# kaushik87599/Melo-GAN

Measured on AMD Instinct MI355X. Metric: piano-roll samples/sec (G+D step), batch=64 128x256 roll, higher is better.
Workload: dtype f32; 1 GPU; cfg2: 128x256 piano-roll, batch=64 per GPU, full G+D+emotion-D step (1 critic update incl. gradient penalty + 1 generator update); global_batch=64, T=256, C=128, parallelism=dp1, graph=True

## Files before the change

### melo-gan_amd/csrc/small_kernels.hip

```cpp
#include "common.h"

namespace {

constexpr int RED_SPLITS = 256;

__device__ __forceinline__ float wave_sum(float v) {
#pragma unroll
    for (int o = 32; o > 0; o >>= 1) v += __shfl_xor(v, o, 64);
    return v;
}

__device__ __forceinline__ float block_sum(float v, float* sh) {
    v = wave_sum(v);
    const int w = threadIdx.x >> 6;
    __syncthreads();
    if ((threadIdx.x & 63) == 0) sh[w] = v;
    __syncthreads();
    float t = 0.f;
    for (int i = 0; i < (int)(blockDim.x >> 6); ++i) t += sh[i];
    return t;
}

template <int MODE>
__global__ __launch_bounds__(256) void colsum_partial_kernel(const float* __restrict__ x, const float* __restrict__ a,
// ... 97 lines not shown
    __shared__ double sh[2][16][FIN_CH];
    const int cx = threadIdx.x & (FIN_CH - 1), g = threadIdx.x / FIN_CH;
    const int c = blockIdx.x * FIN_CH + cx;
    double a = 0.0, b = 0.0;
    if (c < C)
        for (int k = g; k < nsplit; k += 16) {
            a += part[((long)k * 2) * C + c];
            if (want2) b += part[((long)k * 2 + 1) * C + c];
        }
    sh[0][g][cx] = a;
    sh[1][g][cx] = b;
    __syncthreads();
    c_out = c;
    if (g != 0 || c >= C) return false;
    s1 = 0.0;
    s2 = 0.0;
#pragma unroll
    for (int y = 0; y < 16; ++y) {
        s1 += sh[0][y][cx];
        s2 += sh[1][y][cx];
    }
    return true;
}

__global__ __launch_bounds__(256) void colsum_final_kernel(const double* __restrict__ part, int nsplit, int C,
                                                           float* sum, float* sumsq) {
    double s1, s2;
    int c;
    if (!reduce_partials(part, nsplit, C, sumsq != nullptr, s1, s2, c)) return;
    sum[c] = (float)s1;
    if (sumsq) sumsq[c] = (float)s2;
}

__global__ void bn_eval_kernel(const float* __restrict__ z, float* __restrict__ a, long n, int C,
                               const float* __restrict__ gamma, const float* __restrict__ beta,
                               const float* __restrict__ rm, const float* __restrict__ rv, float eps, int act) {
    const long i = (long)blockIdx.x * blockDim.x + threadIdx.x;
    if (i >= n) return;
    const int c = (int)(i % C);
    const float v = (z[i] - rm[c]) / sqrtf(rv[c] + eps) * gamma[c] + beta[c];
    a[i] = mg_act(act, v);
}

__global__ void bn_fold_kernel(const float* gamma, const float* beta, const float* rm, const float* rv,
                               const float* cb, float eps, float* scale, float* shift, int C) {
    const int c = blockIdx.x * blockDim.x + threadIdx.x;
    if (c >= C) return;
    const float s = gamma[c] / sqrtf(rv[c] + eps);
    scale[c] = s;
    shift[c] = beta[c] + ((cb ? cb[c] : 0.f) - rm[c]) * s;
}

constexpr int BNA_THREADS = 1024, BNA_PL = BNA_THREADS / 64;
__device__ __forceinline__ void combine_parts64(const float* __restrict__ part, int np, int C, int c0, double (*sh)[64],
                                                double& mean, double& var) {
    const int cx = threadIdx.x & 63, pl = threadIdx.x >> 6;
    double A = 0.0, Q = 0.0, Bt = 0.0, n = 0.0;
    if (c0 + cx < C) {
        for (int q0 = pl; q0 < np; q0 += 8 * BNA_PL) {
            float va[8], vq[8], vn[8];
#pragma unroll
            for (int j = 0; j < 8; ++j) {
                const int q = q0 + BNA_PL * j;
                const long o = ((long)(q < np ? q : np - 1) * 3) * C + c0 + cx;
                va[j] = part[o];
                vq[j] = part[o + C];
                vn[j] = part[o + 2 * (long)C];
            }
#pragma unroll
            for (int j = 0; j < 8; ++j)
                if (q0 + BNA_PL * j < np && vn[j] > 0.f) {
                    const double a = (double)va[j], c = (double)vn[j];
                    A += a; Q += (double)vq[j]; Bt += a * a / c; n += c;
                }
        }
    }
    __syncthreads();
    sh[pl][cx] = A; sh[BNA_PL + pl][cx] = Q; sh[2 * BNA_PL + pl][cx] = Bt; sh[3 * BNA_PL + pl][cx] = n;
    __syncthreads();
    A = Q = Bt = n = 0.0;
#pragma unroll
    for (int l = 0; l < BNA_PL; ++l) {
        A += sh[l][cx]; Q += sh[BNA_PL + l][cx]; Bt += sh[2 * BNA_PL + l][cx]; n += sh[3 * BNA_PL + l][cx];
    }
    mean = n > 0.0 ? A / n : 0.0;
    double m2 = Q + (Bt - A * mean);
    if (m2 < 0.0) m2 = 0.0;
    var = n > 0.0 ? m2 / n : 0.0;
}

__device__ __forceinline__ void combine_colsum64(const double* __restrict__ part, int np, int C, int c0, long R, double (*sh)[64],
                                                 double& mean, double& var) {
    const int cx = threadIdx.x & 63, pl = threadIdx.x >> 6;
    double A = 0.0, Q = 0.0;
    if (c0 + cx < C)
        for (int q0 = pl; q0 < np; q0 += 8 * BNA_PL) {
            double va[8], vq[8];
#pragma unroll
            for (int j = 0; j < 8; ++j) {
                const int q = q0 + BNA_PL * j;
                const long o = ((long)(q < np ? q : np - 1) * 2) * C + c0 + cx;
                va[j] = part[o];
                vq[j] = part[o + C];
            }
#pragma unroll
            for (int j = 0; j < 8; ++j)
                if (q0 + BNA_PL * j < np) { A += va[j]; Q += vq[j]; }
        }
    __syncthreads();
    sh[pl][cx] = A; sh[BNA_PL + pl][cx] = Q;
    __syncthreads();
    A = Q = 0.0;
#pragma unroll
    for (int l = 0; l < BNA_PL; ++l) { A += sh[l][cx]; Q += sh[BNA_PL + l][cx]; }
    mean = A / (double)R;
    var = Q / (double)R - mean * mean;
    if (var < 0.0) var = 0.0;
}

template <typename PT>
__global__ __launch_bounds__(BNA_THREADS) void bn_parts_apply_kernel(const PT* __restrict__ part, int np, int groups, long R, int C,
                                                             float momentum, float eps, float* running_mean, float* running_var,
                                                             float* save_mean, float* save_invstd, const float* __restrict__ z,
                                                             float* __restrict__ a, const float* __restrict__ gamma,
                                                             const float* __restrict__ beta, int act, long rows_per, int al16) {
    __shared__ double sh[4 * BNA_PL][64];
    __shared__ float s_mean[64], s_istd[64];
    const int c0 = blockIdx.x * 64, cx = threadIdx.x & 63;
    const int g = blockIdx.z;
    if (blockIdx.y == 0 && g == 0) {
        for (int gg = 0; gg < groups; ++gg) {
            double mean, var;
            if constexpr (sizeof(PT) == 4) combine_parts64(part + (long)gg * np * 3 * C, np, C, c0, sh, mean, var);
            else combine_colsum64(part + (long)gg * (RED_SPLITS + 1) * 2 * C, np, C, c0, R, sh, mean, var);
            if (threadIdx.x < 64 && c0 + cx < C) {
                const float mf = (float)mean, isf = (float)(1.0 / sqrt(var + (double)eps));
                save_mean[(long)gg * C + c0 + cx] = mf;
                save_invstd[(long)gg * C + c0 + cx] = isf;
                if (gg == 0) { s_mean[cx] = mf; s_istd[cx] = isf; }
                if (running_mean) {
                    const double unb = R > 1 ? var * (double)R / (double)(R - 1) : var;
                    running_mean[c0 + cx] = (float)((1.0 - momentum) * running_mean[c0 + cx] + momentum * mean);
                    running_var[c0 + cx] = (float)((1.0 - momentum) * running_var[c0 + cx] + momentum * unb);
                }
            }
        }
    } else {
        double mean, var;
        if constexpr (sizeof(PT) == 4) combine_parts64(part + (long)g * np * 3 * C, np, C, c0, sh, mean, var);
        else combine_colsum64(part + (long)g * (RED_SPLITS + 1) * 2 * C, np, C, c0, R, sh, mean, var);
        if (threadIdx.x < 64 && c0 + cx < C) {
            s_mean[cx] = (float)mean;
            s_istd[cx] = (float)(1.0 / sqrt(var + (double)eps));
        }
    }
    __syncthreads();
    const int cq = threadIdx.x & 15, ry = threadIdx.x >> 4;
    constexpr int RYN = BNA_THREADS / 16;
    const int c = c0 + 4 * cq;
    if (c >= C) return;
    const long r0 = (long)blockIdx.y * rows_per;
    long r1 = r0 + rows_per;
    if (r1 > R) r1 = R;
    const bool vec = al16 && (c + 3 < C);
    double mu[4], is[4], ga[4], be[4];
#pragma unroll
    for (int e = 0; e < 4; ++e) {
        const bool in = c + e < C;
        mu[e] = (double)s_mean[4 * cq + e];
        is[e] = (double)s_istd[4 * cq + e];
        ga[e] = in ? (double)gamma[c + e] : 0.0;
        be[e] = in ? (double)beta[c + e] : 0.0;
    }
    const float* zg = z + (long)g * R * C;
    float* ag = a + (long)g * R * C;
    for (long r = r0 + ry; r < r1; r += RYN) {
        const long i = r * C + c;
        if (vec) {
            const float4 t = *reinterpret_cast<const float4*>(zg + i);
            const float zv[4] = {t.x, t.y, t.z, t.w};
            float o[4];
#pragma unroll
            for (int e = 0; e < 4; ++e) o[e] = (float)(((double)zv[e] - mu[e]) * is[e] * ga[e] + be[e]);
            if (act == MG_ACT_RELU) {
#pragma unroll
                for (int e = 0; e < 4; ++e) o[e] = mg_act(MG_ACT_RELU, o[e]);
            } else if (act != MG_ACT_NONE) {
#pragma unroll
                for (int e = 0; e < 4; ++e) o[e] = mg_act(act, o[e]);
            }
            *reinterpret_cast<float4*>(ag + i) = make_float4(o[0], o[1], o[2], o[3]);
        } else {
            for (int e = 0; e < 4; ++e)
                if (c + e < C) ag[i + e] = mg_act(act, (float)(((double)zg[i + e] - mu[e]) * is[e] * ga[e] + be[e]));
        }
    }
}

template <typename PT>
__global__ __launch_bounds__(BNA_THREADS) void bn_bwd_parts_apply_kernel(const PT* __restrict__ part, int nsplit, int C, long R,
                                                                 const float* __restrict__ da, const float* __restrict__ a,
                                                                 const float* __restrict__ z, float* __restrict__ dz,
                                                                 const float* __restrict__ gamma, const float* __restrict__ beta,
                                                                 const float* __restrict__ mean, const float* __restrict__ invstd,
                                                                 float* dgamma, float* dbeta, int act, long rows_per, int al16) {
    __shared__ double sh[2 * BNA_PL][64];
    __shared__ double s1[64], s2[64];
    const int c0 = blockIdx.x * 64, cx = threadIdx.x & 63, pl = threadIdx.x >> 6;
    {
        double t1 = 0.0, t2 = 0.0;
        if (c0 + cx < C)
            for (int q0 = pl; q0 < nsplit; q0 += 8 * BNA_PL) {
                PT va[8], vb[8];
#pragma unroll
                for (int j = 0; j < 8; ++j) {
                    const int q = q0 + BNA_PL * j;
                    const long o = ((long)(q < nsplit ? q : nsplit - 1) * 2) * C + c0 + cx;
                    va[j] = part[o];
                    vb[j] = part[o + C];
                }
#pragma unroll
                for (int j = 0; j < 8; ++j)
                    if (q0 + BNA_PL * j < nsplit) { t1 += (double)va[j]; t2 += (double)vb[j]; }
            }
        sh[pl][cx] = t1;
        sh[BNA_PL + pl][cx] = t2;
        __syncthreads();
        if (threadIdx.x < 64) {
            double u1 = 0.0, u2 = 0.0;
#pragma unroll
            for (int l = 0; l < BNA_PL; ++l) { u1 += sh[l][cx]; u2 += sh[BNA_PL + l][cx]; }
            s1[cx] = u1;
            s2[cx] = u2;
            if (blockIdx.y == 0 && c0 + cx < C) {
                dbeta[c0 + cx] = (float)u1;
                dgamma[c0 + cx] = (float)u2;
            }
        }
        __syncthreads();
    }
    const int cq = threadIdx.x & 15, ry = threadIdx.x >> 4;
    constexpr int RYN = BNA_THREADS / 16;
    const int c = c0 + 4 * cq;
    if (c >= C) return;
    const long r0 = (long)blockIdx.y * rows_per;
    long r1 = r0 + rows_per;
    if (r1 > R) r1 = R;
    const bool vec = al16 && (c + 3 < C);
    const bool pre = act == MG_ACT_GELU;
    const double invR = 1.0 / (double)R;
    double mu[4], is[4], ga[4], be[4], k1[4], k2[4];
#pragma unroll
    for (int e = 0; e < 4; ++e) {
        const bool in = c + e < C;
        mu[e] = in ? (double)mean[c + e] : 0.0;
        is[e] = in ? (double)invstd[c + e] : 0.0;
        ga[e] = in ? (double)gamma[c + e] : 0.0;
        be[e] = (in && pre) ? (double)beta[c + e] : 0.0;
        k1[e] = s1[4 * cq + e];
        k2[e] = s2[4 * cq + e];
    }
    for (long r = r0 + ry; r < r1; r += RYN) {
        const long i = r * C + c;
        float dv[4] = {0, 0, 0, 0}, av[4] = {0, 0, 0, 0}, zv[4] = {0, 0, 0, 0};
        if (vec) {
            const float4 t = *reinterpret_cast<const float4*>(da + i);
            const float4 ta = *reinterpret_cast<const float4*>(a + i);
            const float4 tz = *reinterpret_cast<const float4*>(z + i);
            dv[0] = t.x; dv[1] = t.y; dv[2] = t.z; dv[3] = t.w;
            av[0] = ta.x; av[1] = ta.y; av[2] = ta.z; av[3] = ta.w;
            zv[0] = tz.x; zv[1] = tz.y; zv[2] = tz.z; zv[3] = tz.w;
        } else {
            for (int e = 0; e < 4; ++e)
                if (c + e < C) { dv[e] = da[i + e]; av[e] = a[i + e]; zv[e] = z[i + e]; }
        }
        float o[4];
#pragma unroll
        for (int e = 0; e < 4; ++e) {
            const double xh = ((double)zv[e] - mu[e]) * is[e];
            const float ref = pre ? (float)(xh * ga[e] + be[e]) : av[e];
            const double dy = (double)(dv[e] * mg_act_grad(act, ref));
            o[e] = (float)(ga[e] * is[e] * (dy - k1[e] * invR - xh * k2[e] * invR));
        }
        if (vec) *reinterpret_cast<float4*>(dz + i) = make_float4(o[0], o[1], o[2], o[3]);
        else
            for (int e = 0; e < 4; ++e)
                if (c + e < C) dz[i + e] = o[e];
    }
}

__global__ __launch_bounds__(256) void meanT_fwd_kernel(const float* __restrict__ a, float* __restrict__ h, int T, int C) {
    const int b = blockIdx.y;
    const int cq = threadIdx.x & 15, ry = threadIdx.x >> 4;
    const int c0 = blockIdx.x * 64 + 4 * cq;
    __shared__ float sh[16][65];
    float s[4] = {0.f, 0.f, 0.f, 0.f};
    const bool vec = ((C & 3) == 0) && ((((uintptr_t)a) & 15) == 0);
    if (c0 < C) {
        for (int t = ry; t < T; t += 16) {
            const float* row = a + ((long)b * T + t) * C + c0;
            if (vec) {
                const float4 v = *reinterpret_cast<const float4*>(row);
                s[0] += v.x; s[1] += v.y; s[2] += v.z; s[3] += v.w;
            } else {
                for (int e = 0; e < 4; ++e)
                    if (c0 + e < C) s[e] += row[e];
            }
        }
    }
#pragma unroll
    for (int e = 0; e < 4; ++e) sh[ry][4 * cq + e] = s[e];
    __syncthreads();
    if (threadIdx.x < 64) {
        const int c = blockIdx.x * 64 + threadIdx.x;
        if (c < C) {
            float t = 0.f;
#pragma unroll
            for (int y = 0; y < 16; ++y) t += sh[y][threadIdx.x];
            h[(long)b * C + c] = t / (float)T;
        }
    }
}

template <bool VEC>
__global__ void meanT_bwd_kernel(const float* __restrict__ dh, float* __restrict__ dz, long n, int T, int C,
                                 const float* __restrict__ gref, int gact, const float* __restrict__ gscale,
                                 const float* __restrict__ mean_src, float* mean_out, int mean_n, float mean_scale) {
    constexpr int NV = VEC ? 4 : 1;
    if (mean_out && blockIdx.x == gridDim.x - 1) {
        __shared__ float sh[16];
        float r = 0.f;
        for (int b = threadIdx.x; b < mean_n; b += blockDim.x) r += mean_src[b];
        r = block_sum(r, sh);
        if (threadIdx.x == 0) mean_out[0] = mean_scale * r / (float)mean_n;
        return;
    }
    const long i = ((long)blockIdx.x * blockDim.x + threadIdx.x) * NV;
    if (i >= n) return;
    const int c = (int)(i % C);
    const long b = i / ((long)T * C);
// ... 703 lines not shown
#pragma unroll
    for (int u = 0; u < AUG_UNROLL; ++u) {
        const int e = e0 + u * AUG_THREADS;
        if (e < n) d[e] = v[u];
    }
}

__global__ __launch_bounds__(256) void weighted_order_kernel(const double* __restrict__ cdf, long n, int64_t* __restrict__ order,
                                                             long m, unsigned long long seed, unsigned long long epoch) {
    const long i = (long)blockIdx.x * blockDim.x + threadIdx.x;
    if (i >= m) return;
    unsigned c[4];
    aug_draw(c, (unsigned)i, AUG_ORDER, epoch, seed);
    const unsigned long long bits = ((unsigned long long)(c[0] >> 5) << 26) | (unsigned long long)(c[1] >> 6);
    const double x = (double)bits * (1.0 / 9007199254740992.0) * cdf[n - 1];
    long lo = 0, hi = n - 1;
    while (lo < hi) {
        const long mid = (lo + hi) >> 1;
        if (cdf[mid] > x) hi = mid;
        else lo = mid + 1;
    }
    order[i] = lo < n - 1 ? lo : n - 1;
}

__global__ __launch_bounds__(64) void ed_metrics_acc_kernel(const float* __restrict__ logits, const int64_t* __restrict__ labels,
                                                            const float* __restrict__ loss, int rows, int C,
                                                            float* __restrict__ acc) {
    float hits = 0.f;
    for (int r = threadIdx.x; r < rows; r += 64) {
        const float* z = logits + (long)r * C;
        float mx = z[0];
        int am = 0;
        for (int j = 1; j < C; ++j) {
            const float v = z[j];
            if (v > mx || (isnan(v) && !isnan(mx))) { mx = v; am = j; }
        }
        hits += (long)am == labels[r] ? 1.f : 0.f;
    }
    hits = wave_sum(hits);
    if (threadIdx.x == 0) {
        acc[0] = __fadd_rn(acc[0], __fmul_rn(loss[0], (float)rows));
        acc[1] = __fadd_rn(acc[1], hits);
    }
}

__global__ void adam_advance_kernel(double* state, double beta1, double beta2) {
    if (threadIdx.x == 0 && blockIdx.x == 0) {
        if (state[0] == 0.0) { state[1] = 1.0; state[2] = 1.0; }
        state[0] += 1.0;
        state[1] *= beta1;
        state[2] *= beta2;
    }
}
struct WqTable { mg_wq_entry e[MG_MAX_WQ_ENTRIES]; int n; long lo, hi; };

__global__ void adam_apply_kernel(float* __restrict__ p, const float* __restrict__ g, float* __restrict__ m,
                                  float* __restrict__ v, long n, float lr, float beta1, float beta2, float eps,
                                  float wd, const double* __restrict__ state, float grad_scale,
                                  const float* __restrict__ gs_dev, unsigned long long* bump, const WqTable wq) {
    const long i = (long)blockIdx.x * blockDim.x + threadIdx.x;
    if (bump && i == 0) bump[0] += 1;
    if (i >= n) return;
    const double bc1 = 1.0 - state[1];
    const double bc2 = 1.0 - state[2];
    const float step_size = (float)((double)lr / bc1);
    const float bc2_sqrt = (float)sqrt(bc2);
    float gs = grad_scale;
    if (gs_dev) gs *= gs_dev[0];
    const float gi = g[i] * gs;
    float pi = p[i];
    if (wd != 0.f) pi *= (1.f - lr * wd);
    const float mi = m[i] + (gi - m[i]) * (1.f - beta1);
    const float vi = v[i] * beta2 + (1.f - beta2) * gi * gi;
    m[i] = mi;
    v[i] = vi;
    const float denom = sqrtf(vi) / bc2_sqrt + eps;
    pi = pi - step_size * (mi / denom);
    p[i] = pi;
    if (i >= wq.lo && i < wq.hi) {
        for (int t = 0; t < wq.n; ++t) {
            const mg_wq_entry& e = wq.e[t];
            const long L = i - e.start;
            if (L < 0 || L >= (long)e.N * e.Cc * e.K) continue;
            const int k = (int)(L % e.K);
            const long r = L / e.K;
            int nn, c;
            if (e.w_sc == e.K) { nn = (int)(r / e.Cc); c = (int)(r % e.Cc); }
            else { c = (int)(r / e.N); nn = (int)(r % e.N); }
            e.dst[((long)((c >> 2) * e.K + k) * e.N + nn) * 4 + (c & 3)] = pi;
        }
    }
}

__global__ __launch_bounds__(1024) void sumsq_partial_kernel(const float* __restrict__ g, long n, float* part) {
    __shared__ float sh[16];
    float s = 0.f;
    for (long i = (long)blockIdx.x * blockDim.x + threadIdx.x; i < n; i += (long)gridDim.x * blockDim.x)
        s += g[i] * g[i];
    s = block_sum(s, sh);
    if (threadIdx.x == 0) part[blockIdx.x] = s;
}
__global__ __launch_bounds__(256) void norm_clip_final_kernel(const float* part, int nparts, float max_norm, float* out) {
    __shared__ double shd[256];
    double t = 0.0;
    for (int i = threadIdx.x; i < nparts; i += 256) t += (double)part[i];
    shd[threadIdx.x] = t;
    __syncthreads();
    for (int o = 128; o > 0; o >>= 1) {
        if ((int)threadIdx.x < o) shd[threadIdx.x] += shd[threadIdx.x + o];
        __syncthreads();
    }
    if (threadIdx.x == 0) {
        const double s = shd[0];
        const float nrm = (float)sqrt(s);
        out[0] = nrm;
        const float c = max_norm / (nrm + 1e-6f);
        out[1] = c < 1.f ? c : 1.f;
    }
}

struct SnJobs { mg_sn_job j[MG_MAX_SN_JOBS]; int n; };

__global__ __launch_bounds__(1024) void spectral_norm_fwd_kernel(const SnJobs J, int power_iter, float eps) {
    __shared__ float sh[16];
    const mg_sn_job jb = J.j[blockIdx.x];
    const int R = jb.rows, Cc = jb.cols;
    const float* __restrict__ W = jb.w_orig;
    float* u = jb.u;
    float* v = jb.v;
    const int tid = threadIdx.x, lane = tid & 63, wave = tid >> 6;
    if (power_iter) {
        for (int j = tid; j < Cc; j += 1024) {
            float acc = 0.f;
            for (int i = 0; i < R; ++i) acc += W[(long)i * Cc + j] * u[i];
            v[j] = acc;
        }
        __threadfence_block();
        __syncthreads();
        float q = 0.f;
        for (int j = tid; j < Cc; j += 1024) q += v[j] * v[j];
        q = block_sum(q, sh);
        const float sv = 1.f / fmaxf(sqrtf(q), eps);
        for (int j = tid; j < Cc; j += 1024) v[j] *= sv;
        __threadfence_block();
// ... 538 lines not shown
    const char* pname[3] = {"dropout_prob", "pitch_shift_prob", "note_dropout"};
    for (int i = 0; i < 3; ++i)
        MG_CHECK_ARG(probs[i] >= 0.f && probs[i] <= 1.f, "mg_stage_augment: %s must be in [0, 1]", pname[i]);
    const float sig[4] = {aug->noise_std, aug->tempo_jitter, aug->velocity_jitter, aug->timing_jitter};
    const char* sname[4] = {"noise_std", "tempo_jitter", "velocity_jitter", "timing_jitter"};
    for (int i = 0; i < 4; ++i)
        MG_CHECK_ARG(sig[i] >= 0.f && sig[i] < INFINITY, "mg_stage_augment: %s must be finite and not negative", sname[i]);
    MG_CHECK_ARG(aug->pitch_shift >= 0 && aug->pitch_shift <= (1 << 20), "mg_stage_augment: pitch_shift must be in 0..2^20");
    const int Q = note_dim / 4;
    const long bx = mg_cdiv((long)T * Q, AUG_THREADS * AUG_UNROLL);
    hipLaunchKernelGGL(stage_augment_kernel, dim3((unsigned)bx, (unsigned)n_rows), dim3(AUG_THREADS), 0, ST,
                       reinterpret_cast<const float4*>(notes), labels, src_rows, T, Q, reinterpret_cast<float4*>(notes_out),
                       labels_out, n_rows, order, order_len, reinterpret_cast<const unsigned long long*>(counter),
                       reinterpret_cast<const unsigned long long*>(base), reinterpret_cast<const unsigned long long*>(serial_base),
                       rule, *aug);
    MG_CHECK_LAUNCH("stage_augment");
    return MG_OK;
}

int mg_weighted_order(const double* cdf, long n, int64_t* order, long m, uint64_t seed, uint64_t epoch, mg_stream_t stream) {
    MG_CHECK_ARG(cdf && order, "mg_weighted_order: null cdf / order");
    MG_CHECK_ARG(n > 0, "mg_weighted_order: n must be positive");
    MG_CHECK_ARG(m > 0 && m <= 0x7FFFFFFFL, "mg_weighted_order: m must be in 1..2^31-1");
    hipLaunchKernelGGL(weighted_order_kernel, dim3((unsigned)mg_cdiv(m, 256)), dim3(256), 0, ST, cdf, n, order, m,
                       (unsigned long long)seed, (unsigned long long)epoch);
    MG_CHECK_LAUNCH("weighted_order");
    return MG_OK;
}

int mg_ed_metrics_acc(const float* logits, const int64_t* labels, const float* loss, int rows, int n_classes, float* acc,
                      mg_stream_t stream) {
    MG_CHECK_ARG(logits && labels && loss && acc, "mg_ed_metrics_acc: null logits / labels / loss / acc");
    MG_CHECK_ARG(rows > 0 && rows < (1 << 24), "mg_ed_metrics_acc: rows must be in 1..2^24-1");
    MG_CHECK_ARG(n_classes >= 1, "mg_ed_metrics_acc: n_classes must be positive");
    hipLaunchKernelGGL(ed_metrics_acc_kernel, dim3(1), dim3(64), 0, ST, logits, labels, loss, rows, n_classes, acc);
    MG_CHECK_LAUNCH("ed_metrics_acc");
    return MG_OK;
}

int mg_adam_flat(float* p, const float* g, float* m, float* v, long n, float lr, float beta1, float beta2,
                 float eps, float weight_decay, double* state, float grad_scale, const float* gs_dev,
                 int state_ticked, uint64_t* rng_step, const mg_wq_entry* table, int n_table, mg_stream_t stream) {
    MG_CHECK_ARG(p && g && m && v && state && n > 0, "mg_adam_flat: bad args");
    MG_CHECK_ARG(n_table >= 0 && n_table <= MG_MAX_WQ_ENTRIES && (n_table == 0 || table), "mg_adam_flat: bad table");
    WqTable t{};
    t.n = n_table;
    t.lo = n; t.hi = 0;
    for (int i = 0; i < n_table; ++i) {
        const mg_wq_entry& e = table[i];
        const long cnt = (long)e.N * e.Cc * e.K;
        MG_CHECK_ARG(e.dst && e.N > 0 && e.Cc > 0 && e.Cc % 4 == 0 && e.K > 0 && e.start >= 0 && e.start + cnt <= n &&
                     ((e.w_sc == e.K && e.w_sn == e.Cc * e.K) || (e.w_sn == e.K && e.w_sc == e.N * e.K)),
                     "mg_adam_flat: table entry %d is not a dense (N,C,K) or (C,N,K) tensor inside the flat buffer", i);
        t.e[i] = e;
        if (e.start < t.lo) t.lo = e.start;
        if (e.start + cnt > t.hi) t.hi = e.start + cnt;
    }
    if (!state_ticked)
        hipLaunchKernelGGL(adam_advance_kernel, dim3(1), dim3(64), 0, ST, state, (double)beta1, (double)beta2);
    hipLaunchKernelGGL(adam_apply_kernel, dim3(nblk(n)), dim3(256), 0, ST, p, g, m, v, n, lr, beta1, beta2, eps,
                       weight_decay, (const double*)state, grad_scale, gs_dev, (unsigned long long*)rng_step, t);
    MG_CHECK_LAUNCH("adam_flat");
    return MG_OK;
}

static int sn_jobs(const mg_sn_job* jobs, int n_jobs, bool bwd, SnJobs& J, const char* who) {
    MG_CHECK_ARG(jobs && n_jobs > 0 && n_jobs <= MG_MAX_SN_JOBS, "%s: 1..%d jobs", who, MG_MAX_SN_JOBS);
    J.n = n_jobs;
    for (int i = 0; i < n_jobs; ++i) {
        const mg_sn_job& q = jobs[i];
        MG_CHECK_ARG(q.w_eff && q.u && q.v && q.sigma && q.rows > 0 && q.cols > 0 && (bwd ? q.dw != nullptr : q.w_orig != nullptr),
                     "%s: job %d: null tensor or empty shape", who, i);
        J.j[i] = q;
    }
    return MG_OK;
}

int mg_spectral_norm_fwd(const mg_sn_job* jobs, int n_jobs, int power_iterations, float eps, mg_stream_t stream) {
    SnJobs J{};
    if (int rc = sn_jobs(jobs, n_jobs, false, J, "mg_spectral_norm_fwd")) return rc;
    MG_CHECK_ARG(power_iterations == 0 || power_iterations == 1, "mg_spectral_norm_fwd: 0 (eval) or 1 power iteration");
    hipLaunchKernelGGL(spectral_norm_fwd_kernel, dim3((unsigned)n_jobs), dim3(1024), 0, ST, J, power_iterations, eps);
    MG_CHECK_LAUNCH("spectral_norm_fwd");
    return MG_OK;
}

int mg_spectral_norm_bwd(const mg_sn_job* jobs, int n_jobs, mg_stream_t stream) {
    SnJobs J{};
    if (int rc = sn_jobs(jobs, n_jobs, true, J, "mg_spectral_norm_bwd")) return rc;
    hipLaunchKernelGGL(spectral_norm_bwd_kernel, dim3((unsigned)n_jobs), dim3(1024), 0, ST, J);
    MG_CHECK_LAUNCH("spectral_norm_bwd");
    return MG_OK;
}

size_t mg_grad_norm_workspace_bytes(long n) { return 1024 * sizeof(float); }

int mg_grad_norm_clip(const float* g, long n, float max_norm, float* out, void* work, size_t work_bytes,
                      mg_stream_t stream) {
    MG_CHECK_ARG(g && out && n > 0, "mg_grad_norm_clip: bad args");
    if (!work || work_bytes < mg_grad_norm_workspace_bytes(n)) { mg_set_error("mg_grad_norm_clip: workspace too small"); return MG_EWORK; }
    int nparts = (int)mg_cdiv(n, 1024 * 8);
    if (nparts > 1024) nparts = 1024;
    if (nparts < 1) nparts = 1;
    hipLaunchKernelGGL(sumsq_partial_kernel, dim3(nparts), dim3(1024), 0, ST, g, n, (float*)work);
    hipLaunchKernelGGL(norm_clip_final_kernel, dim3(1), dim3(256), 0, ST, (const float*)work, nparts, max_norm, out);
    MG_CHECK_LAUNCH("grad_norm_clip");
    return MG_OK;
}

int mg_reparam_fwd(const float* mu, const float* logvar, const float* eps, float* z, long n, mg_stream_t stream) {
    MG_CHECK_ARG(mu && logvar && eps && z && n > 0, "mg_reparam_fwd: bad args");
    hipLaunchKernelGGL(reparam_kernel, dim3(nblk(n)), dim3(256), 0, ST, mu, logvar, eps, z, n);
    MG_CHECK_LAUNCH("reparam");
    return MG_OK;
// ... 30 lines not shown
```

Baseline: 80690 samples/s.

## Prefetch BN partials and inputs early, restructure BN apply/backward and vectorize Adam

The BN stats-combine-and-apply kernels now issue their first partial-sum loads and first activation rows before the cross-wave reduction, and stage gamma/beta in shared memory. The running-statistics update stays in registers for all groups and is written once. The row loops software-prefetch the next row. Adam gets an optional 4-wide vectorized path for large buffers and replaces div/mod in the weight-layout copy with precomputed magic-number division. The goal is to hide global-load latency and cut integer-division cost, at the price of more registers and branching.

Result: no change. 81360 samples/s (median of 6 runs) (+0.8%).

```diff
diff --git a/melo-gan_amd/csrc/small_kernels.hip b/melo-gan_amd/csrc/small_kernels.hip
--- a/melo-gan_amd/csrc/small_kernels.hip
+++ b/melo-gan_amd/csrc/small_kernels.hip
@@ -173,32 +173,62 @@
 }
 
 constexpr int BNA_THREADS = 1024, BNA_PL = BNA_THREADS / 64;
-__device__ __forceinline__ void combine_parts64(const float* __restrict__ part, int np, int C, int c0, double (*sh)[64],
-                                                double& mean, double& var) {
-    const int cx = threadIdx.x & 63, pl = threadIdx.x >> 6;
+struct Parts3 { float a[8], q[8], n[8]; };
+template <typename PT> struct Parts2 { PT a[8], q[8]; };
+template <typename T>
+__device__ __forceinline__ T parts_at(const T* row, int col) {
+    return *reinterpret_cast<const T*>(reinterpret_cast<const char*>(row) + (unsigned)col * (unsigned)sizeof(T));
+}
+__device__ __forceinline__ void parts_load(const float* __restrict__ part, int np, int C, int col, int q0, Parts3& v) {
+#pragma unroll
+    for (int j = 0; j < 8; ++j) {
+        const int q = q0 + BNA_PL * j;
+        const float* row = part + (long)(q < np ? q : np - 1) * 3 * C;
+        v.a[j] = parts_at(row, col);
+        v.q[j] = parts_at(row + C, col);
+        v.n[j] = parts_at(row + 2 * (long)C, col);
+    }
+}
+template <typename PT>
+__device__ __forceinline__ void parts_load(const PT* __restrict__ part, int np, int C, int col, int q0, Parts2<PT>& v) {
+#pragma unroll
+    for (int j = 0; j < 8; ++j) {
+        const int q = q0 + BNA_PL * j;
+        const PT* row = part + (long)(q < np ? q : np - 1) * 2 * C;
+        v.a[j] = parts_at(row, col);
+        v.q[j] = parts_at(row + C, col);
+    }
+}
+__device__ __forceinline__ void parts_acc(const Parts3& v, int np, int q0, double& A, double& Q, double& Bt, double& n) {
+#pragma unroll
+    for (int j = 0; j < 8; ++j)
+        if (q0 + BNA_PL * j < np && v.n[j] > 0.f) {
+            const double a = (double)v.a[j], c = (double)v.n[j];
+            A += a; Q += (double)v.q[j]; Bt += a * a / c; n += c;
+        }
+}
+template <typename PT>
+__device__ __forceinline__ void parts_acc(const Parts2<PT>& v, int np, int q0, double& A, double& Q) {
+#pragma unroll
+    for (int j = 0; j < 8; ++j)
+        if (q0 + BNA_PL * j < np) { A += (double)v.a[j]; Q += (double)v.q[j]; }
+}
+
+__device__ __forceinline__ void combine_parts64(const float* __restrict__ part, int np, int C, int col, const Parts3& first,
+                                                double (*sh)[64], double& mean, double& var) {
+    const int cx = threadIdx.x & 63, pl = __builtin_amdgcn_readfirstlane(threadIdx.x >> 6);
     double A = 0.0, Q = 0.0, Bt = 0.0, n = 0.0;
-    if (c0 + cx < C) {
-        for (int q0 = pl; q0 < np; q0 += 8 * BNA_PL) {
-            float va[8], vq[8], vn[8];
-#pragma unroll
-            for (int j = 0; j < 8; ++j) {
-                const int q = q0 + BNA_PL * j;
-                const long o = ((long)(q < np ? q : np - 1) * 3) * C + c0 + cx;
-                va[j] = part[o];
-                vq[j] = part[o + C];
-                vn[j] = part[o + 2 * (long)C];
-            }
-#pragma unroll
-            for (int j = 0; j < 8; ++j)
-                if (q0 + BNA_PL * j < np && vn[j] > 0.f) {
-                    const double a = (double)va[j], c = (double)vn[j];
-                    A += a; Q += (double)vq[j]; Bt += a * a / c; n += c;
-                }
-        }
+    parts_acc(first, np, pl, A, Q, Bt, n);
+    for (int q0 = pl + 8 * BNA_PL; q0 < np; q0 += 8 * BNA_PL) {
+        Parts3 v;
+        parts_load(part, np, C, col, q0, v);
+        parts_acc(v, np, q0, A, Q, Bt, n);
     }
     __syncthreads();
     sh[pl][cx] = A; sh[BNA_PL + pl][cx] = Q; sh[2 * BNA_PL + pl][cx] = Bt; sh[3 * BNA_PL + pl][cx] = n;
     __syncthreads();
+    mean = var = 0.0;
+    if (threadIdx.x >= 64) return;
     A = Q = Bt = n = 0.0;
 #pragma unroll
     for (int l = 0; l < BNA_PL; ++l) {
@@ -210,33 +240,32 @@
     var = n > 0.0 ? m2 / n : 0.0;
 }
 
-__device__ __forceinline__ void combine_colsum64(const double* __restrict__ part, int np, int C, int c0, long R, double (*sh)[64],
-                                                 double& mean, double& var) {
-    const int cx = threadIdx.x & 63, pl = threadIdx.x >> 6;
+__device__ __forceinline__ void combine_colsum64(const double* __restrict__ part, int np, int C, int col, const Parts2<double>& first,
+                                                 long R, double (*sh)[64], double& mean, double& var) {
+    const int cx = threadIdx.x & 63, pl = __builtin_amdgcn_readfirstlane(threadIdx.x >> 6);
     double A = 0.0, Q = 0.0;
-    if (c0 + cx < C)
-        for (int q0 = pl; q0 < np; q0 += 8 * BNA_PL) {
-            double va[8], vq[8];
-#pragma unroll
-            for (int j = 0; j < 8; ++j) {
-                const int q = q0 + BNA_PL * j;
-                const long o = ((long)(q < np ? q : np - 1) * 2) * C + c0 + cx;
-                va[j] = part[o];
-                vq[j] = part[o + C];
-            }
-#pragma unroll
-            for (int j = 0; j < 8; ++j)
-                if (q0 + BNA_PL * j < np) { A += va[j]; Q += vq[j]; }
-        }
+    parts_acc(first, np, pl, A, Q);
+    for (int q0 = pl + 8 * BNA_PL; q0 < np; q0 += 8 * BNA_PL) {
+        Parts2<double> v;
+        parts_load(part, np, C, col, q0, v);
+        parts_acc(v, np, q0, A, Q);
+    }
     __syncthreads();
     sh[pl][cx] = A; sh[BNA_PL + pl][cx] = Q;
     __syncthreads();
+    mean = var = 0.0;
+    if (threadIdx.x >= 64) return;
     A = Q = 0.0;
 #pragma unroll
     for (int l = 0; l < BNA_PL; ++l) { A += sh[l][cx]; Q += sh[BNA_PL + l][cx]; }
     mean = A / (double)R;
     var = Q / (double)R - mean * mean;
     if (var < 0.0) var = 0.0;
+}
+
+__device__ __forceinline__ float bn_running_step(float run, float momentum, double x) {
+#pragma clang fp contract(off)
+    return (float)__builtin_fma((double)momentum, x, (1.0 - momentum) * (double)run);
 }
 
 template <typename PT>
@@ -246,74 +275,110 @@
                                                              float* __restrict__ a, const float* __restrict__ gamma,
                                                              const float* __restrict__ beta, int act, long rows_per, int al16) {
     __shared__ double sh[4 * BNA_PL][64];
-    __shared__ float s_mean[64], s_istd[64];
-    const int c0 = blockIdx.x * 64, cx = threadIdx.x & 63;
+    __shared__ float s_mean[64], s_istd[64], s_ga[64], s_be[64];
+    using Parts = typename std::conditional<sizeof(PT) == 4, Parts3, Parts2<double>>::type;
+    const int c0 = blockIdx.x * 64, cx = threadIdx.x & 63, pl = __builtin_amdgcn_readfirstlane(threadIdx.x >> 6);
     const int g = blockIdx.z;
-    if (blockIdx.y == 0 && g == 0) {
-        for (int gg = 0; gg < groups; ++gg) {
-            double mean, var;
-            if constexpr (sizeof(PT) == 4) combine_parts64(part + (long)gg * np * 3 * C, np, C, c0, sh, mean, var);
-            else combine_colsum64(part + (long)gg * (RED_SPLITS + 1) * 2 * C, np, C, c0, R, sh, mean, var);
-            if (threadIdx.x < 64 && c0 + cx < C) {
-                const float mf = (float)mean, isf = (float)(1.0 / sqrt(var + (double)eps));
-                save_mean[(long)gg * C + c0 + cx] = mf;
-                save_invstd[(long)gg * C + c0 + cx] = isf;
-                if (gg == 0) { s_mean[cx] = mf; s_istd[cx] = isf; }
-                if (running_mean) {
-                    const double unb = R > 1 ? var * (double)R / (double)(R - 1) : var;
-                    running_mean[c0 + cx] = (float)((1.0 - momentum) * running_mean[c0 + cx] + momentum * mean);
-                    running_var[c0 + cx] = (float)((1.0 - momentum) * running_var[c0 + cx] + momentum * unb);
-                }
-            }
-        }
-    } else {
-        double mean, var;
-        if constexpr (sizeof(PT) == 4) combine_parts64(part + (long)g * np * 3 * C, np, C, c0, sh, mean, var);
-        else combine_colsum64(part + (long)g * (RED_SPLITS + 1) * 2 * C, np, C, c0, R, sh, mean, var);
-        if (threadIdx.x < 64 && c0 + cx < C) {
-            s_mean[cx] = (float)mean;
-            s_istd[cx] = (float)(1.0 / sqrt(var + (double)eps));
-        }
-    }
-    __syncthreads();
+    const bool pub = blockIdx.y == 0 && g == 0;
+    const long gstride = sizeof(PT) == 4 ? (long)np * 3 * C : (long)(RED_SPLITS + 1) * 2 * C;
     const int cq = threadIdx.x & 15, ry = threadIdx.x >> 4;
     constexpr int RYN = BNA_THREADS / 16;
     const int c = c0 + 4 * cq;
-    if (c >= C) return;
     const long r0 = (long)blockIdx.y * rows_per;
     long r1 = r0 + rows_per;
     if (r1 > R) r1 = R;
+    const long rf = r0 + ry;
+    const float* zg = z + (long)g * R * C;
+    float* ag = a + (long)g * R * C;
+
+    float zv[4];
+    {
+        const long rc = rf < R ? rf : R - 1;
+        if (al16) {
+            const float4 t = *reinterpret_cast<const float4*>(zg + rc * C + (c < C ? c : C - 4));
+            zv[0] = t.x; zv[1] = t.y; zv[2] = t.z; zv[3] = t.w;
+        } else {
+#pragma unroll
+            for (int e = 0; e < 4; ++e) zv[e] = zg[rc * C + (c + e < C ? c + e : C - 1)];
+        }
+    }
+    const int col = c0 + cx < C ? c0 + cx : C - 1;
+    Parts p0, p1;
+    const bool two = pub && groups > 1;
+    parts_load(part + (long)g * gstride, np, C, col, pl, p0);
+    const float gav = gamma[col], bev = beta[col];
+    float rm = 0.f, rv = 0.f;
+    if (pub && running_mean) { rm = running_mean[col]; rv = running_var[col]; }
+    if (two) parts_load(part + gstride, np, C, col, pl, p1);
+    __builtin_amdgcn_sched_barrier(0);
+
+    auto finish = [&](int gg, const Parts& first, bool publish) {
+        double mean, var;
+        if constexpr (sizeof(PT) == 4) combine_parts64(part + (long)gg * gstride, np, C, col, first, sh, mean, var);
+        else combine_colsum64(part + (long)gg * gstride, np, C, col, first, R, sh, mean, var);
+        if (threadIdx.x < 64 && c0 + cx < C) {
+            const float mf = (float)mean, isf = (float)(1.0 / sqrt(var + (double)eps));
+            if (gg == g) { s_mean[cx] = mf; s_istd[cx] = isf; }
+            if (publish) {
+                save_mean[(long)gg * C + c0 + cx] = mf;
+                save_invstd[(long)gg * C + c0 + cx] = isf;
+                if (running_mean) {
+                    const double unb = R > 1 ? var * (double)R / (double)(R - 1) : var;
+                    rm = bn_running_step(rm, momentum, mean);
+                    rv = bn_running_step(rv, momentum, unb);
+                }
+            }
+        }
+    };
+    finish(g, p0, pub);
+    if (two) {
+        finish(1, p1, true);
+        for (int gg = 2; gg < groups; ++gg) {
+            parts_load(part + (long)gg * gstride, np, C, col, pl, p1);
+            finish(gg, p1, true);
+        }
+    }
+    if (pub && running_mean && threadIdx.x < 64 && c0 + cx < C) {
+        running_mean[c0 + cx] = rm;
+        running_var[c0 + cx] = rv;
+    }
+    if (threadIdx.x < 64) { s_ga[cx] = gav; s_be[cx] = bev; }
+    __syncthreads();
+    if (c >= C) return;
     const bool vec = al16 && (c + 3 < C);
     double mu[4], is[4], ga[4], be[4];
 #pragma unroll
     for (int e = 0; e < 4; ++e) {
-        const bool in = c + e < C;
         mu[e] = (double)s_mean[4 * cq + e];
         is[e] = (double)s_istd[4 * cq + e];
-        ga[e] = in ? (double)gamma[c + e] : 0.0;
-        be[e] = in ? (double)beta[c + e] : 0.0;
-    }
-    const float* zg = z + (long)g * R * C;
-    float* ag = a + (long)g * R * C;
-    for (long r = r0 + ry; r < r1; r += RYN) {
+        ga[e] = (double)s_ga[4 * cq + e];
+        be[e] = (double)s_be[4 * cq + e];
+    }
+    for (long r = rf; r < r1; r += RYN) {
         const long i = r * C + c;
-        if (vec) {
-            const float4 t = *reinterpret_cast<const float4*>(zg + i);
-            const float zv[4] = {t.x, t.y, t.z, t.w};
-            float o[4];
-#pragma unroll
-            for (int e = 0; e < 4; ++e) o[e] = (float)(((double)zv[e] - mu[e]) * is[e] * ga[e] + be[e]);
-            if (act == MG_ACT_RELU) {
-#pragma unroll
-                for (int e = 0; e < 4; ++e) o[e] = mg_act(MG_ACT_RELU, o[e]);
-            } else if (act != MG_ACT_NONE) {
-#pragma unroll
-                for (int e = 0; e < 4; ++e) o[e] = mg_act(act, o[e]);
+        float o[4];
+#pragma unroll
+        for (int e = 0; e < 4; ++e) o[e] = (float)(((double)zv[e] - mu[e]) * is[e] * ga[e] + be[e]);
+        if (act == MG_ACT_RELU) {
+#pragma unroll
+            for (int e = 0; e < 4; ++e) o[e] = mg_act(MG_ACT_RELU, o[e]);
+        } else if (act != MG_ACT_NONE) {
+#pragma unroll
+            for (int e = 0; e < 4; ++e) o[e] = mg_act(act, o[e]);
+        }
+        if (vec) *reinterpret_cast<float4*>(ag + i) = make_float4(o[0], o[1], o[2], o[3]);
+        else
+            for (int e = 0; e < 4; ++e)
+                if (c + e < C) ag[i + e] = o[e];
+        if (r + RYN < r1) {
+            const long j = i + (long)RYN * C;
+            if (vec) {
+                const float4 t = *reinterpret_cast<const float4*>(zg + j);
+                zv[0] = t.x; zv[1] = t.y; zv[2] = t.z; zv[3] = t.w;
+            } else {
+                for (int e = 0; e < 4; ++e)
+                    if (c + e < C) zv[e] = zg[j + e];
             }
-            *reinterpret_cast<float4*>(ag + i) = make_float4(o[0], o[1], o[2], o[3]);
-        } else {
-            for (int e = 0; e < 4; ++e)
-                if (c + e < C) ag[i + e] = mg_act(act, (float)(((double)zg[i + e] - mu[e]) * is[e] * ga[e] + be[e]));
         }
     }
 }
@@ -327,23 +392,50 @@
                                                                  float* dgamma, float* dbeta, int act, long rows_per, int al16) {
     __shared__ double sh[2 * BNA_PL][64];
     __shared__ double s1[64], s2[64];
-    const int c0 = blockIdx.x * 64, cx = threadIdx.x & 63, pl = threadIdx.x >> 6;
+    __shared__ float s_mu[64], s_is[64], s_ga[64], s_be[64];
+    const int c0 = blockIdx.x * 64, cx = threadIdx.x & 63, pl = __builtin_amdgcn_readfirstlane(threadIdx.x >> 6);
+    const int cq = threadIdx.x & 15, ry = threadIdx.x >> 4;
+    constexpr int RYN = BNA_THREADS / 16;
+    const int c = c0 + 4 * cq;
+    const long r0 = (long)blockIdx.y * rows_per;
+    long r1 = r0 + rows_per;
+    if (r1 > R) r1 = R;
+    const long rf = r0 + ry;
+    const bool pre = act == MG_ACT_GELU;
+
+    float dv[4], av[4], zv[4];
+    {
+        const long rc = rf < R ? rf : R - 1;
+        if (al16) {
+            const long o = rc * C + (c < C ? c : C - 4);
+            const float4 t = *reinterpret_cast<const float4*>(da + o);
+            const float4 ta = *reinterpret_cast<const float4*>(a + o);
+            const float4 tz = *reinterpret_cast<const float4*>(z + o);
+            dv[0] = t.x; dv[1] = t.y; dv[2] = t.z; dv[3] = t.w;
+            av[0] = ta.x; av[1] = ta.y; av[2] = ta.z; av[3] = ta.w;
+            zv[0] = tz.x; zv[1] = tz.y; zv[2] = tz.z; zv[3] = tz.w;
+        } else {
+#pragma unroll
+            for (int e = 0; e < 4; ++e) {
+                const long o = rc * C + (c + e < C ? c + e : C - 1);
+                dv[e] = da[o]; av[e] = a[o]; zv[e] = z[o];
+            }
+        }
+    }
+    const int col = c0 + cx < C ? c0 + cx : C - 1;
+    Parts2<PT> p0;
+    parts_load(part, nsplit, C, col, pl, p0);
+    const float muv = mean[col], isv = invstd[col], gav = gamma[col];
+    const float bev = (pre ? beta : gamma)[col];
+    __builtin_amdgcn_sched_barrier(0);
     {
         double t1 = 0.0, t2 = 0.0;
-        if (c0 + cx < C)
-            for (int q0 = pl; q0 < nsplit; q0 += 8 * BNA_PL) {
-                PT va[8], vb[8];
-#pragma unroll
-                for (int j = 0; j < 8; ++j) {
-                    const int q = q0 + BNA_PL * j;
-                    const long o = ((long)(q < nsplit ? q : nsplit - 1) * 2) * C + c0 + cx;
-                    va[j] = part[o];
-                    vb[j] = part[o + C];
-                }
-#pragma unroll
-                for (int j = 0; j < 8; ++j)
-                    if (q0 + BNA_PL * j < nsplit) { t1 += (double)va[j]; t2 += (double)vb[j]; }
-            }
+        parts_acc(p0, nsplit, pl, t1, t2);
+        for (int q0 = pl + 8 * BNA_PL; q0 < nsplit; q0 += 8 * BNA_PL) {
+            Parts2<PT> v;
+            parts_load(part, nsplit, C, col, q0, v);
+            parts_acc(v, nsplit, q0, t1, t2);
+        }
         sh[pl][cx] = t1;
         sh[BNA_PL + pl][cx] = t2;
         __syncthreads();
@@ -357,44 +449,25 @@
                 dbeta[c0 + cx] = (float)u1;
                 dgamma[c0 + cx] = (float)u2;
             }
+            s_mu[cx] = muv; s_is[cx] = isv; s_ga[cx] = gav; s_be[cx] = pre ? bev : 0.f;
         }
         __syncthreads();
     }
-    const int cq = threadIdx.x & 15, ry = threadIdx.x >> 4;
-    constexpr int RYN = BNA_THREADS / 16;
-    const int c = c0 + 4 * cq;
     if (c >= C) return;
-    const long r0 = (long)blockIdx.y * rows_per;
-    long r1 = r0 + rows_per;
-    if (r1 > R) r1 = R;
     const bool vec = al16 && (c + 3 < C);
-    const bool pre = act == MG_ACT_GELU;
     const double invR = 1.0 / (double)R;
     double mu[4], is[4], ga[4], be[4], k1[4], k2[4];
 #pragma unroll
     for (int e = 0; e < 4; ++e) {
-        const bool in = c + e < C;
-        mu[e] = in ? (double)mean[c + e] : 0.0;
-        is[e] = in ? (double)invstd[c + e] : 0.0;
-        ga[e] = in ? (double)gamma[c + e] : 0.0;
-        be[e] = (in && pre) ? (double)beta[c + e] : 0.0;
+        mu[e] = (double)s_mu[4 * cq + e];
+        is[e] = (double)s_is[4 * cq + e];
+        ga[e] = (double)s_ga[4 * cq + e];
+        be[e] = (double)s_be[4 * cq + e];
         k1[e] = s1[4 * cq + e];
         k2[e] = s2[4 * cq + e];
     }
-    for (long r = r0 + ry; r < r1; r += RYN) {
+    for (long r = rf; r < r1; r += RYN) {
         const long i = r * C + c;
-        float dv[4] = {0, 0, 0, 0}, av[4] = {0, 0, 0, 0}, zv[4] = {0, 0, 0, 0};
-        if (vec) {
-            const float4 t = *reinterpret_cast<const float4*>(da + i);
-            const float4 ta = *reinterpret_cast<const float4*>(a + i);
-            const float4 tz = *reinterpret_cast<const float4*>(z + i);
-            dv[0] = t.x; dv[1] = t.y; dv[2] = t.z; dv[3] = t.w;
-            av[0] = ta.x; av[1] = ta.y; av[2] = ta.z; av[3] = ta.w;
-            zv[0] = tz.x; zv[1] = tz.y; zv[2] = tz.z; zv[3] = tz.w;
-        } else {
-            for (int e = 0; e < 4; ++e)
-                if (c + e < C) { dv[e] = da[i + e]; av[e] = a[i + e]; zv[e] = z[i + e]; }
-        }
         float o[4];
 #pragma unroll
         for (int e = 0; e < 4; ++e) {
@@ -407,6 +480,20 @@
         else
             for (int e = 0; e < 4; ++e)
                 if (c + e < C) dz[i + e] = o[e];
+        if (r + RYN < r1) {
+            const long j = i + (long)RYN * C;
+            if (vec) {
+                const float4 t = *reinterpret_cast<const float4*>(da + j);
+                const float4 ta = *reinterpret_cast<const float4*>(a + j);
+                const float4 tz = *reinterpret_cast<const float4*>(z + j);
+                dv[0] = t.x; dv[1] = t.y; dv[2] = t.z; dv[3] = t.w;
+                av[0] = ta.x; av[1] = ta.y; av[2] = ta.z; av[3] = ta.w;
+                zv[0] = tz.x; zv[1] = tz.y; zv[2] = tz.z; zv[3] = tz.w;
+            } else {
+                for (int e = 0; e < 4; ++e)
+                    if (c + e < C) { dv[e] = da[j + e]; av[e] = a[j + e]; zv[e] = z[j + e]; }
+            }
+        }
     }
 }
 
@@ -1216,44 +1303,99 @@
         state[2] *= beta2;
     }
 }
-struct WqTable { mg_wq_entry e[MG_MAX_WQ_ENTRIES]; int n; long lo, hi; };
-
-__global__ void adam_apply_kernel(float* __restrict__ p, const float* __restrict__ g, float* __restrict__ m,
+struct WqEntry {
+    float* dst;
+    long start;
+    unsigned long long mK, m2;
+    unsigned cnt, d2;
+    int N, K, nck;
+};
+struct WqTable { WqEntry e[MG_MAX_WQ_ENTRIES]; int n; long lo, hi; };
+static unsigned long long wq_mul(unsigned d) { return d == 1 ? 0ull : ~0ull / d + 1; }
+__device__ __forceinline__ unsigned wq_div(unsigned a, unsigned long long M) {
+    const unsigned long long t = (M >> 32) * a + (((M & 0xffffffffull) * a) >> 32);
+    return M ? (unsigned)(t >> 32) : a;
+}
+template <int EPT>
+__device__ __forceinline__ void wq_copy(const WqTable& wq, long i, int cnt, const float (&pv)[4]) {
+    for (int t = 0; t < wq.n; ++t) {
+        const WqEntry e = wq.e[t];
+        const long L0 = i - e.start;
+        if (L0 + cnt <= 0 || L0 >= (long)e.cnt) continue;
+#pragma unroll
+        for (int j = 0; j < EPT; ++j) {
+            const long L = L0 + j;
+            if (j >= cnt || L < 0 || L >= (long)e.cnt) continue;
+            const unsigned r = wq_div((unsigned)L, e.mK), k = (unsigned)L - r * (unsigned)e.K;
+            const unsigned hi = wq_div(r, e.m2), lo = r - hi * e.d2;
+            const int nn = (int)(e.nck ? hi : lo), c = (int)(e.nck ? lo : hi);
+            e.dst[((long)((c >> 2) * e.K + (int)k) * e.N + nn) * 4 + (c & 3)] = pv[j];
+        }
+    }
+}
+
+struct AdamK { float lr, beta1, beta2, eps, wd, step_size, bc2_sqrt, gs; };
+__device__ __forceinline__ void adam_one(const AdamK& k, float g, float& p, float& m, float& v) {
+#pragma clang fp contract(off)
+    const float gi = g * k.gs;
+    float pi = p;
+    if (k.wd != 0.f) pi *= __builtin_fmaf(-k.lr, k.wd, 1.f);
+    const float mi = __builtin_fmaf(1.f - k.beta1, __builtin_fmaf(g, k.gs, -m), m);
+    const float vi = __builtin_fmaf(gi, (1.f - k.beta2) * gi, v * k.beta2);
+    m = mi;
+    v = vi;
+    const float denom = sqrtf(vi) / k.bc2_sqrt + k.eps;
+    p = __builtin_fmaf(-(mi / denom), k.step_size, pi);
+}
+
+template <int EPT>
+__global__ __launch_bounds__(256) void adam_apply_kernel(float* __restrict__ p, const float* __restrict__ g, float* __restrict__ m,
                                   float* __restrict__ v, long n, float lr, float beta1, float beta2, float eps,
                                   float wd, const double* __restrict__ state, float grad_scale,
-                                  const float* __restrict__ gs_dev, unsigned long long* bump, const WqTable wq) {
-    const long i = (long)blockIdx.x * blockDim.x + threadIdx.x;
-    if (bump && i == 0) bump[0] += 1;
+                                  const float* __restrict__ gs_dev, unsigned long long* bump, int al16, const WqTable wq) {
+    const long q = (long)blockIdx.x * blockDim.x + threadIdx.x;
+    if (bump && q == 0) bump[0] += 1;
+    const long i = EPT * q;
     if (i >= n) return;
-    const double bc1 = 1.0 - state[1];
-    const double bc2 = 1.0 - state[2];
-    const float step_size = (float)((double)lr / bc1);
-    const float bc2_sqrt = (float)sqrt(bc2);
-    float gs = grad_scale;
-    if (gs_dev) gs *= gs_dev[0];
-    const float gi = g[i] * gs;
-    float pi = p[i];
-    if (wd != 0.f) pi *= (1.f - lr * wd);
-    const float mi = m[i] + (gi - m[i]) * (1.f - beta1);
-    const float vi = v[i] * beta2 + (1.f - beta2) * gi * gi;
-    m[i] = mi;
-    v[i] = vi;
-    const float denom = sqrtf(vi) / bc2_sqrt + eps;
-    pi = pi - step_size * (mi / denom);
-    p[i] = pi;
-    if (i >= wq.lo && i < wq.hi) {
-        for (int t = 0; t < wq.n; ++t) {
-            const mg_wq_entry& e = wq.e[t];
-            const long L = i - e.start;
-            if (L < 0 || L >= (long)e.N * e.Cc * e.K) continue;
-            const int k = (int)(L % e.K);
-            const long r = L / e.K;
-            int nn, c;
-            if (e.w_sc == e.K) { nn = (int)(r / e.Cc); c = (int)(r % e.Cc); }
-            else { c = (int)(r / e.N); nn = (int)(r % e.N); }
-            e.dst[((long)((c >> 2) * e.K + k) * e.N + nn) * 4 + (c & 3)] = pi;
-        }
-    }
+    const bool vec = EPT == 4 && al16 && i + 3 < n;
+    const int cnt = n - i < EPT ? (int)(n - i) : EPT;
+    const double st1 = state[1], st2 = state[2];
+    const float gsv = (gs_dev ? gs_dev : g)[0];
+    float gv[4], pv[4], mv[4], vv[4];
+    if (vec) {
+        const float4 tg = *reinterpret_cast<const float4*>(g + i), tp = *reinterpret_cast<const float4*>(p + i);
+        const float4 tm = *reinterpret_cast<const float4*>(m + i), tv = *reinterpret_cast<const float4*>(v + i);
+        gv[0] = tg.x; gv[1] = tg.y; gv[2] = tg.z; gv[3] = tg.w;
+        pv[0] = tp.x; pv[1] = tp.y; pv[2] = tp.z; pv[3] = tp.w;
+        mv[0] = tm.x; mv[1] = tm.y; mv[2] = tm.z; mv[3] = tm.w;
+        vv[0] = tv.x; vv[1] = tv.y; vv[2] = tv.z; vv[3] = tv.w;
+    } else {
+#pragma unroll
+        for (int e = 0; e < EPT; ++e) {
+            const long j = e < cnt ? i + e : i;
+            gv[e] = g[j]; pv[e] = p[j]; mv[e] = m[j]; vv[e] = v[j];
+        }
+    }
+    AdamK k;
+    k.lr = lr; k.beta1 = beta1; k.beta2 = beta2; k.eps = eps; k.wd = wd;
+    const double bc1 = 1.0 - st1;
+    const double bc2 = 1.0 - st2;
+    k.step_size = (float)((double)lr / bc1);
+    k.bc2_sqrt = (float)sqrt(bc2);
+    k.gs = grad_scale;
+    if (gs_dev) k.gs *= gsv;
+#pragma unroll
+    for (int e = 0; e < EPT; ++e) adam_one(k, gv[e], pv[e], mv[e], vv[e]);
+    if (vec) {
+        *reinterpret_cast<float4*>(m + i) = make_float4(mv[0], mv[1], mv[2], mv[3]);
+        *reinterpret_cast<float4*>(v + i) = make_float4(vv[0], vv[1], vv[2], vv[3]);
+        *reinterpret_cast<float4*>(p + i) = make_float4(pv[0], pv[1], pv[2], pv[3]);
+    } else {
+#pragma unroll
+        for (int e = 0; e < EPT; ++e)
+            if (e < cnt) { m[i + e] = mv[e]; v[i + e] = vv[e]; p[i + e] = pv[e]; }
+    }
+    if (i + cnt > wq.lo && i < wq.hi) wq_copy<EPT>(wq, i, cnt, pv);
 }
 
 __global__ __launch_bounds__(1024) void sumsq_partial_kernel(const float* __restrict__ g, long n, float* part) {
@@ -1898,14 +2040,24 @@
         MG_CHECK_ARG(e.dst && e.N > 0 && e.Cc > 0 && e.Cc % 4 == 0 && e.K > 0 && e.start >= 0 && e.start + cnt <= n &&
                      ((e.w_sc == e.K && e.w_sn == e.Cc * e.K) || (e.w_sn == e.K && e.w_sc == e.N * e.K)),
                      "mg_adam_flat: table entry %d is not a dense (N,C,K) or (C,N,K) tensor inside the flat buffer", i);
-        t.e[i] = e;
+        MG_CHECK_ARG(cnt <= 0xFFFFFFFFL, "mg_adam_flat: table entry %d has 2^32 elements or more", i);
+        WqEntry& d = t.e[i];
+        d.dst = e.dst; d.start = e.start; d.cnt = (unsigned)cnt; d.N = e.N; d.K = e.K;
+        d.nck = e.w_sc == e.K;
+        d.d2 = (unsigned)(d.nck ? e.Cc : e.N);
+        d.mK = wq_mul((unsigned)e.K); d.m2 = wq_mul(d.d2);
         if (e.start < t.lo) t.lo = e.start;
         if (e.start + cnt > t.hi) t.hi = e.start + cnt;
     }
     if (!state_ticked)
         hipLaunchKernelGGL(adam_advance_kernel, dim3(1), dim3(64), 0, ST, state, (double)beta1, (double)beta2);
-    hipLaunchKernelGGL(adam_apply_kernel, dim3(nblk(n)), dim3(256), 0, ST, p, g, m, v, n, lr, beta1, beta2, eps,
-                       weight_decay, (const double*)state, grad_scale, gs_dev, (unsigned long long*)rng_step, t);
+    const int al16 = ((((uintptr_t)p | (uintptr_t)g | (uintptr_t)m | (uintptr_t)v) & 15) == 0);
+    if (n >= 4L * 256 * 2048)
+        hipLaunchKernelGGL(adam_apply_kernel<4>, dim3(nblk(mg_cdiv(n, 4))), dim3(256), 0, ST, p, g, m, v, n, lr, beta1, beta2, eps,
+                           weight_decay, (const double*)state, grad_scale, gs_dev, (unsigned long long*)rng_step, al16, t);
+    else
+        hipLaunchKernelGGL(adam_apply_kernel<1>, dim3(nblk(n)), dim3(256), 0, ST, p, g, m, v, n, lr, beta1, beta2, eps,
+                           weight_decay, (const double*)state, grad_scale, gs_dev, (unsigned long long*)rng_step, al16, t);
     MG_CHECK_LAUNCH("adam_flat");
     return MG_OK;
 }
```
